# NekoImageLand/retto

Hardware: AMD Instinct MI355X
Metric: images/sec end-to-end PP-OCRv4 det+rec @960x960 (higher is better)
Workload: dtype f32; 1 GPU; C3: PP-OCRv4 mobile det+cls+rec full pipeline, batch=32 pages of 960x960 per GPU, 32 planted lines/page (planted DB map drives box extraction; det net fully executed, checksum 1.46374e+07); pages resident in HBM when the timed region starts; weights=seeded synthetic, PP-OCRv4 mobile shapes, networks=mobile/f32 f32 mobile/f32, parallelism=dp1 (pages sharded, no per-step collective), batches_in_flight=2

## Files before the change

### retto_amd/csrc/api_debug.cpp

```cpp
#include <cmath>
#include <cstdio>
#include <cstdlib>
#include <cstring>

#include "api_internal.h"

using namespace rt;

namespace {
using nh::half_t;

std::vector<half_t> pack_conv16_weights(const float* wt, int cout, int cin, int kh, int kw, int cin_pad) {
  const int npad = round_up(cout, 32), nslab = (cin_pad + nh::KS - 1) / nh::KS;
  std::vector<half_t> hw((size_t)nslab * kh * kw * npad * nh::KS, (half_t)0.f);
  for (int n = 0; n < cout; n++)
    for (int k = 0; k < cin; k++)
      for (int t = 0; t < kh * kw; t++)
        hw[(((size_t)(k / nh::KS) * kh * kw + t) * npad + n) * nh::KS + k % nh::KS] = (half_t)wt[((size_t)n * cin + k) * kh * kw + t];
  return hw;
}

inline uint64_t xorshift64(uint64_t& s) { s ^= s << 13; s ^= s >> 7; s ^= s << 17; return s; }

template <typename F>
// ... 234 lines not shown
    if (ctc >= 0) { DevBufs::download(idx_out, didx, (size_t)M); DevBufs::download(prob_out, dprob, (size_t)M); }
    plan_out[0] = (int)plan.kernel; plan_out[1] = plan.nt; plan_out[2] = plan.kg; plan_out[3] = plan.se; plan_out[4] = plan.bf;
  });
}

RT_API int rt_debug_dwconv(rt_session* s, const float* x, const int* heights, const int* widths, int n_img, int C, int Cp, int K,
                           int sh, int sw, const float* w, const float* bias, int act, int has_lab, float lab_a, float lab_c,
                           int pooled, int form, float* out, float* partial_out, long long partial_cap, float* mean_out,
                           int* info_out) {
  RT_REQUIRE(s && x && heights && widths && w && bias && out && info_out, s, "rt_debug_dwconv: null argument");
  RT_REQUIRE(n_img > 0 && C > 0 && Cp >= C && Cp % 4 == 0 && (K == 3 || K == 5) && sh >= 1 && sh <= 2 && sw >= 1 && sw <= 2 &&
                 act >= ACT_NONE && act <= ACT_SIGMOID && (form == 0 || form == 1),
             s, "rt_debug_dwconv: bad shape");
  RT_REQUIRE(!pooled || (partial_out && mean_out), s, "rt_debug_dwconv: pooled without buffers for the sums");
  for (int i = 0; i < n_img; i++) RT_REQUIRE(heights[i] > 0 && widths[i] > 0, s, "rt_debug_dwconv: empty image");
  const Ragged gi(heights, widths, n_img), go = gi.down(sh, sw);
  RT_REQUIRE(gi.total * Cp < (1ll << 30), s, "rt_debug_dwconv: too large");
  RestoreInt keep_form(nn::g_dw_sweep);
  nn::g_dw_sweep = form ? 4 : 0;
  const nn::DwPlan plan = nn::dw_plan(K, sh, sw, Cp, go.maxH, go.maxW, pooled != 0);
  const int chunks = pooled ? plan.chunks : 0, strip_R = pooled ? plan.R : 0, spb = pooled ? plan.spb : 0;
  const size_t npart = (size_t)n_img * chunks * Cp;
  RT_REQUIRE(!pooled || (long long)npart <= partial_cap, s, "rt_debug_dwconv: partial_out is too small");
  return guarded(s, [&] {
    RT_HIP_CHECK(hipSetDevice(s->device));
    DevBufs bufs;
    const size_t nout = (size_t)(go.total + 64) * Cp;
    const float *dx = bufs.upload(x, (size_t)gi.total * Cp), *dw = bufs.upload(w, (size_t)K * K * Cp), *db = bufs.upload(bias, (size_t)Cp);
    const ImgGeom *dgi = gi.upload(bufs), *dgo = go.upload(bufs);
    float* dy = bufs.canary<float>(nout, s->st);
    float* dpart = pooled ? bufs.canary<float>(npart, s->st) : nullptr;
    float* dmean = pooled ? bufs.alloc<float>((size_t)n_img * Cp) : nullptr;
    nn::dwconv(s->st, plan, dx, dgi, dgo, n_img, Cp, C, dw, db, act, has_lab, lab_a, lab_c, dy, dpart);
    if (pooled)
      nn::se_fc_from_dw(s->st, dpart, dgo, n_img, chunks, strip_R, spb, C, Cp, nullptr, nullptr, nullptr, nullptr, 0, 0.f, 0, dmean);
    RT_HIP_CHECK(hipStreamSynchronize(s->st));
    DevBufs::download(out, dy, nout);
    if (pooled) { DevBufs::download(partial_out, dpart, npart); DevBufs::download(mean_out, dmean, (size_t)n_img * Cp); }
    info_out[0] = chunks; info_out[1] = strip_R; info_out[2] = spb;
    info_out[3] = plan.kernel == nn::DwKernel::sweep ? 1 : 0;
  });
}

RT_API int rt_debug_attention(rt_session* s, const float* qkv, long long rows, const int* tokens, int n_lines, int heads, float* out) {
  RT_REQUIRE(s && qkv && tokens && out, s, "rt_debug_attention: null argument");
  RT_REQUIRE(rows > 0 && rows < (1ll << 30) && n_lines > 0 && heads > 0 && heads <= 64, s, "rt_debug_attention: bad shape");
  for (int i = 0; i < n_lines; i++) RT_REQUIRE(tokens[i] > 0, s, "rt_debug_attention: a line without tokens");
  const Ragged lines(tokens, n_lines);
  RT_REQUIRE(lines.total == rows, s, "rt_debug_attention: the lines' tokens do not add up to rows");
  return guarded(s, [&] {
    RT_HIP_CHECK(hipSetDevice(s->device));
    const int hd = 15, C = heads * hd;
    DevBufs bufs;
    const float* dq = bufs.upload(qkv, (size_t)rows * 3 * C);
    float* dout = bufs.zeroed<float>((size_t)rows * C);
    nn::attention(s->st, dq, lines.upload(bufs), n_lines, lines.maxW, heads, hd, dout);
    RT_HIP_CHECK(hipStreamSynchronize(s->st));
    DevBufs::download(out, dout, (size_t)rows * C);
  });
}

static LcBlock debug_lc_block(WeightStore& ws, int cin, int cout, int sh, int sw, const float* dw_w, const float* dw_bias, const float* pw_w,
                              const float* pw_bias, int dw_act, const Lab& dw_lab, const Lab& pw_lab) {
  LcBlock b;
  b.dw = pack_dw(ws, dw_w, dw_bias, cin, 3); b.dw_lab = dw_lab; b.dw_act = dw_act;
  b.pw = pack_conv(ws, pw_w, pw_bias, cout, cin, 1, 1); b.pw_lab = pw_lab;
  b.sh = sh; b.sw = sw; b.cin = cin; b.cout = cout;
  return b;
}
static float* debug_lc_mid(DevBufs& bufs, hipStream_t st, const LcBlock& b, const Level& Lo) {
  if (lc_block_plan(b, Lo).route != nn::LC_UNFUSED) return nullptr;
  const size_t nmid = (size_t)(Lo.total + 256) * b.dw.Cp;
  float* dy1 = bufs.alloc<float>(nmid);
  RT_HIP_CHECK(hipMemsetAsync(dy1, 0, nmid * sizeof(float), st));
  return dy1;
}

RT_API int rt_debug_lc_block(rt_session* s, const float* x, const int* heights, const int* widths, int n_img, int cin, int cout,
                             int sh, int sw, const float* dw_w, const float* dw_bias, const float* pw_w, const float* pw_bias,
                             int dw_act, int dw_has_lab, float dw_a, float dw_c, int pw_has_lab, float pw_a, float pw_c, int form,
                             float* out, int* info_out) {
  RT_REQUIRE(s && x && heights && widths && dw_w && dw_bias && pw_w && pw_bias && out && info_out, s, "rt_debug_lc_block: null argument");
  RT_REQUIRE(n_img > 0 && n_img <= RT_MAX_GRID_Y && cin > 0 && cout > 0 && chan_pitch(cin) == round_up(cin, 4) && sh >= 1 && sh <= 2 &&
                 sw >= 1 && sw <= 2 && dw_act >= ACT_NONE && dw_act <= ACT_SIGMOID && (form == 0 || form == 1 || form == 3),
             s, "rt_debug_lc_block: bad shape");
  const int Cp = chan_pitch(cin), ldy = chan_pitch(cout);
  std::vector<std::pair<int, int>> hw;
  for (int i = 0; i < n_img; i++) {
    RT_REQUIRE(heights[i] > 0 && widths[i] > 0, s, "rt_debug_lc_block: empty image");
    hw.push_back({heights[i], widths[i]});
  }
  Level Li = make_level(hw), Lo = down_level(Li, sh, sw);
  RT_REQUIRE(Li.total * Cp < (1ll << 30) && Lo.total * ldy < (1ll << 30), s, "rt_debug_lc_block: too large");
  return guarded(s, [&] {
    s->begin_call();
    WeightStore ws;
    const LcBlock b = debug_lc_block(ws, cin, cout, sh, sw, dw_w, dw_bias, pw_w, pw_bias, dw_act, Lab{dw_has_lab, dw_a, dw_c}, Lab{pw_has_lab, pw_a, pw_c});
    DevBufs bufs;
    RestoreInt keep_form(nn::g_lc_wave);
    nn::g_lc_wave = form;
    RunCtx c = s->ctx(&s->arena);
    upload_levels(c, {&Li, &Lo});
    const size_t nin = (size_t)Li.total * Cp, nout = (size_t)(Lo.total + 64) * ldy;
    const float* dx = bufs.upload(x, nin);
    float* dy = bufs.canary<float>(nout, s->st);
    run_lc(c, b, dx, Li, Lo, dy, debug_lc_mid(bufs, s->st, b, Lo));
    RT_HIP_CHECK(hipStreamSynchronize(s->st));
    DevBufs::download(out, dy, nout);
    info_out[0] = (int)lc_block_plan(b, Lo).route;
  });
}

RT_API int rt_debug_dw_plan(int K, int sh, int sw, int Cp, int maxHo, int maxWo, int pooled, int form, int* plan_out) {
  rt_session* const none = nullptr;
  RT_REQUIRE(plan_out, none, "rt_debug_dw_plan: null argument");
  RT_REQUIRE(Cp > 0 && Cp % 4 == 0 && maxHo > 0 && maxWo > 0 && (form == 0 || form == 1), none, "rt_debug_dw_plan: bad shape");
  RestoreInt keep_form(nn::g_dw_sweep);
  nn::g_dw_sweep = form ? 4 : 0;
  const nn::DwPlan p = nn::dw_plan(K, sh, sw, Cp, maxHo, maxWo, pooled != 0);
  const int f[8] = {(int)p.kernel, p.inst, p.R, p.lanes, p.spb, p.chunks, (int)p.grid_x, (int)p.grid_z};
  memcpy(plan_out, f, sizeof f);
  return RT_OK;
}

RT_API int rt_debug_lc_wide(rt_session* s, const float* x, const int* heights, const int* widths, int n_img, int K, int cin, int cout,
                            int sh, int sw, const float* dw_w, const float* dw_bias, const float* pw_w, const float* pw_bias, int dw_act,
                            int dw_has_lab, float dw_a, float dw_c, int pw_has_lab, float pw_a, float pw_c, const float* fc1_w,
                            const float* fc1_b, const float* fc2_w, const float* fc2_b, int dw_form, float* out, long long out_len,
                            float* y1_out, long long y1_len, float* scale_out, long long scale_len, int* info_out) {
  RT_REQUIRE(x && heights && widths && dw_w && dw_bias && pw_w && pw_bias && out && y1_out && info_out, s, "rt_debug_lc_wide: null argument");
  const bool se = fc1_w || fc1_b || fc2_w || fc2_b;
  RT_REQUIRE(!se || (fc1_w && fc1_b && fc2_w && fc2_b && scale_out), s, "rt_debug_lc_wide: a squeeze-excite block needs both FCs and scale_out");
  RT_REQUIRE(n_img > 0 && n_img <= 4096, s, "rt_debug_lc_wide: bad image count");
  RT_REQUIRE(cin > 0 && cin <= 512 && cin % 4 == 0 && cout > 0 && cout <= 960, s, "rt_debug_lc_wide: bad channel counts (cin a multiple of 4 up to 512, cout up to 960)");
  RT_REQUIRE((K == 3 || K == 5) && sh >= 1 && sh <= 2 && sw >= 1 && sw <= 2 && dw_act >= ACT_NONE && dw_act <= ACT_SIGMOID &&
                 (dw_form == 0 || dw_form == 1), s, "rt_debug_lc_wide: no such block (K 3 or 5, strides 1 or 2, dw_form 0 or 1)");
  for (int i = 0; i < n_img; i++)
    RT_REQUIRE(heights[i] > 0 && widths[i] > 0 && heights[i] <= 4096 && widths[i] <= 65536, s, "rt_debug_lc_wide: empty or oversized image");
  const int Cp = chan_pitch(cin), ldy = chan_pitch(cout);
  const Ragged gi(heights, widths, n_img), go = gi.down(sh, sw);
  RT_REQUIRE(gi.total * Cp < (1ll << 28) && go.total * ldy < (1ll << 28), s, "rt_debug_lc_wide: too large");
  const long long out_n = (go.total + 64) * ldy, y1_n = (go.total + 64) * Cp, scale_n = se ? (long long)(n_img + 64) * Cp : 0;
  RT_REQUIRE(out_len == out_n && y1_len == y1_n, s, "rt_debug_lc_wide: out or y1_out has the wrong length");
  RT_REQUIRE(scale_len == scale_n, s, "rt_debug_lc_wide: scale_out has the wrong length");
  RT_REQUIRE(s, s, "rt_debug_lc_wide: null session");
  return guarded(s, [&] {
    s->begin_call();
    WeightStore ws;
    LcBlock b;
    b.dw = pack_dw(ws, dw_w, dw_bias, cin, K); b.dw_lab = Lab{dw_has_lab, dw_a, dw_c}; b.dw_act = dw_act;
    b.se = se;
    if (se) b.sew = get_se(ws, fc1_w, fc1_b, fc2_w, fc2_b, cin, cin / 4);
    b.pw = pack_conv(ws, pw_w, pw_bias, cout, cin, 1, 1); b.pw_lab = Lab{pw_has_lab, pw_a, pw_c};
    b.sh = sh; b.sw = sw; b.cin = cin; b.cout = cout;
    std::vector<std::pair<int, int>> hw;
    for (int i = 0; i < n_img; i++) hw.push_back({heights[i], widths[i]});
    Level Li = make_level(hw), Lo = down_level(Li, sh, sw);
    DevBufs bufs;
    RestoreInt keep_form(nn::g_dw_sweep), keep_variant(nn::g_gemm_variant);
    nn::g_dw_sweep = dw_form ? 4 : 0;
    nn::g_gemm_variant = 0;
    RunCtx c = s->ctx(&s->arena);
    upload_levels(c, {&Li, &Lo});
    const float* dx = bufs.upload(x, (size_t)Li.total * Cp);
    float* dy = bufs.canary<float>((size_t)out_n, s->st);
    float* dy1 = bufs.canary<float>((size_t)(Lo.total + 256) * Cp, s->st);
    const nn::LcPlan plan = lc_block_plan(b, Lo);
    LcTrace tr;
    run_lc(c, b, dx, Li, Lo, dy, dy1, &tr);
    RT_HIP_CHECK(hipStreamSynchronize(s->st));
    DevBufs::download(out, dy, (size_t)out_n);
    DevBufs::download(y1_out, dy1, (size_t)y1_n);
    if (se) {
      const uint32_t cw = RT_DEBUG_CANARY;
      for (long long i = 0; i < scale_n; i++) memcpy(scale_out + i, &cw, 4);
      if (tr.scale) DevBufs::download(scale_out, tr.scale, (size_t)n_img * Cp);
    }
    const bool unfused = plan.route == nn::LC_UNFUSED;
    const int f[16] = {(int)plan.route, unfused ? (int)plan.dw.kernel : 0, unfused ? plan.dw.inst : plan.inst, plan.dw.R, plan.dw.lanes,
                       plan.dw.spb, plan.dw.chunks, (int)plan.dw.grid_x, (int)plan.dw.grid_z, plan.se_rows,
                       unfused ? (int)tr.gemm.kernel : 0, unfused && tr.gemm.se ? 1 : 0, tr.scale ? (tr.scaled_in_place ? 2 : 1) : 0, 0, 0, 0};
    memcpy(info_out, f, sizeof f);
  });
// ... 567 lines not shown
      x_need = gi.total * Cp; out_rows = go.total;
      break;
    case G32_AVGPOOL:
      ldy = ip[1];
      ok = C % 4 == 0 && ldy >= C && ldy <= 16384 && ldy % 4 == 0;
      for (int i = 0; ok && i < n_img; i++) ok = heights[i] >= 3 && widths[i] >= 2;
      if (ok) go = gi.pool(3, 2);
      x_need = gi.total * Cp; out_rows = go.total;
      break;
    case G32_SOFTMAX: case G32_ARGMAX_PROB: case G32_ARGMAX:
      ok = ip[1] >= C && ip[1] <= 16384 && (op == G32_SOFTMAX || idx_out);
      x_need = (long long)n_img * ip[1]; out_rows = n_img; ldy = op == G32_SOFTMAX ? C : 1;
      break;
  }
  RT_REQUIRE(ok, s, "rt_debug_glue32: bad parameters for the op");
  RT_REQUIRE(x_need < (1ll << 28) && out_rows * ldy < (1ll << 28), s, "rt_debug_glue32: too large");
  const long long out_n = (out_rows + 64) * ldy;
  RT_REQUIRE(x_len >= x_need && out_len == out_n, s, "rt_debug_glue32: x is too short or out has the wrong length");
  RT_REQUIRE(out2_n == 0 || (out2 && out2_len == out2_n), s, "rt_debug_glue32: out2 is missing or has the wrong length");
  RT_REQUIRE(s, s, "rt_debug_glue32: null session");
  return guarded(s, [&] {
    RT_HIP_CHECK(hipSetDevice(s->device));
    DevBufs bufs;
    WeightStore ws;
    hipStream_t st = s->st;
    float* dout = bufs.canary<float>((size_t)out_n, st);
    const ImgGeom* dgi = rows_op ? nullptr : gi.upload(bufs);
    switch (op) {
      case G32_SE_SCALE: {
        const SeW se = get_se(ws, w[0], w[1], w[2], w[3], C, Cr);
        float* dx = nullptr;
        if (out2_n) { dx = bufs.canary<float>((size_t)out2_n, st); DevBufs::put(dx, x, (size_t)x_need); }
        else dx = bufs.upload(x, (size_t)x_need);
        float* partial = bufs.alloc<float>((size_t)n_img * nn::pool_chunks(gi.max_pix) * Cp);
        nn::se_scale(st, dx, dgi, n_img, gi.max_pix, se.C, Cp, se.w1, se.b1, se.w2, se.b2, se.Cr, fp[0], ip[2], partial, dout);
        if (out2_n) nn::scale_channels(st, dx, dgi, n_img, gi.max_pix, Cp, dout);
        RT_HIP_CHECK(hipStreamSynchronize(st));
        if (out2_n) DevBufs::download(out2, dx, (size_t)out2_n);
      } break;
      case G32_GLOBAL_MEAN: {
        float* partial = bufs.alloc<float>((size_t)n_img * nn::pool_chunks(gi.max_pix) * Cp);
        nn::global_mean(st, bufs.upload(x, (size_t)x_need), dgi, n_img, gi.max_pix, Cp, partial, dout);
      } break;
      case G32_MAXPOOL: nn::maxpool_2x2(st, bufs.upload(x, (size_t)x_need), dgi, go.upload(bufs), n_img, go.max_pix, Cp, dout); break;
      case G32_AVGPOOL: nn::avgpool_3x2(st, bufs.upload(x, (size_t)x_need), dgi, go.upload(bufs), n_img, go.max_pix, Cp, dout, ldy); break;
      case G32_SOFTMAX: nn::softmax_rows(st, bufs.upload(x, (size_t)x_need), ip[1], n_img, C, dout); break;
      case G32_ARGMAX_PROB: case G32_ARGMAX: {
        int* didx = bufs.canary<int>((size_t)out_n, st);
        const float* dx = bufs.upload(x, (size_t)x_need);
        if (op == G32_ARGMAX_PROB) nn::argmax_prob_rows(st, dx, ip[1], n_img, C, didx, dout);
        else nn::argmax_rows(st, dx, ip[1], n_img, C, didx, dout);
        RT_HIP_CHECK(hipStreamSynchronize(st));
        DevBufs::download(idx_out, didx, (size_t)out_n);
      } break;
    }
    RT_HIP_CHECK(hipStreamSynchronize(st));
    DevBufs::download(out, dout, (size_t)out_n);
  });
}

RT_API int rt_bench_lc(rt_session* s, int n, int h, int w, int cin, int cout, int stride, int form, int iters, float* ms_out, float* maxdiff_out) {
  RT_REQUIRE(s && ms_out && n > 0 && h > 0 && w > 0 && cin > 0 && cout > 0 && (stride == 1 || stride == 2 || stride == 21), s, "rt_bench_lc: bad argument");
  return guarded(s, [&] {
    s->begin_call();
    const int sh = stride == 21 ? 2 : stride, sw = stride == 21 ? 1 : stride;
    std::vector<float> hwd((size_t)cin * 9), hbd(cin), hw((size_t)cout * cin), hb(cout);
    uint32_t st = 777;
    auto rnd = [&]() { st = st * 1664525u + 1013904223u; return ((st >> 8) & 0xffff) / 32768.0f - 1.0f; };
    for (auto& v : hwd) v = rnd() * 0.3f;
    for (auto& v : hw) v = rnd() * 0.1f;
    for (auto& v : hbd) v = rnd() * 0.1f;
    for (auto& v : hb) v = rnd() * 0.2f;
    const bool plain_tail = sh == 2 && sw == 2;
    WeightStore ws;
    const LcBlock blk = debug_lc_block(ws, cin, cout, sh, sw, hwd.data(), hbd.data(), hw.data(), hb.data(), plain_tail ? ACT_NONE : ACT_HSWISH,
                                     Lab{!plain_tail, 0.99f, 0.01f}, Lab{1, 1.01f, 0.02f});
    Level Li = make_level(std::vector<std::pair<int, int>>((size_t)n, {h, w})), Lo = down_level(Li, sh, sw);
    RunCtx c = s->ctx(&s->arena);
    upload_levels(c, {&Li, &Lo});
    const size_t nin = (size_t)Li.total * blk.dw.Cp, nout = (size_t)Lo.total * chan_pitch(cout);
    std::vector<float> hx(nin, 0.f);
    for (size_t p = 0; p < (size_t)Li.total; p++) for (int k = 0; k < cin; k++) hx[p * blk.dw.Cp + k] = rnd();
    DevBufs bufs;
    RestoreInt keep_form(nn::g_lc_wave);
    float *dx = bufs.upload(hx.data(), nin), *dy = bufs.zeroed<float>(nout), *dy0 = bufs.zeroed<float>(nout);
    float* dy1 = nullptr;
    auto run = [&](float* out) {
      if (!dy1) dy1 = debug_lc_mid(bufs, s->st, blk, Lo);
      run_lc(c, blk, dx, Li, Lo, out, dy1);
    };
    nn::g_lc_wave = 0; run(dy0);
    nn::g_lc_wave = form;
    timed_and_compared(s->st, iters, [&] { run(dy); }, dy0, dy, nout, ms_out, maxdiff_out);
  });
}

RT_API int rt_debug_det_tiles(rt_session* s, const uint8_t* rgb_det, int h, int w, float* tile_maps_out, float* page_map_out) {
  RT_REQUIRE(s && rgb_det && page_map_out, s, "rt_debug_det_tiles: null argument");
  return guarded(s, [&] { s->debug_det_tiles(rgb_det, h, w, tile_maps_out, page_map_out); });
}
RT_API int rt_debug_rec_windows(rt_session* s, const float* nchw, int n, const int* widths, int32_t* unit_idx_out, float* unit_prob_out,
                                float* unit_z5_out, int32_t* line_idx_out, float* line_prob_out, float* line_z5_out) {
  RT_REQUIRE(s && nchw && widths && n > 0, s, "rt_debug_rec_windows: bad argument");
  return guarded(s, [&] {
    s->debug_rec_windows(nchw, n, widths, unit_idx_out, unit_prob_out, unit_z5_out, line_idx_out, line_prob_out, line_z5_out);
  });
}
RT_API int rt_debug_arena_high_water(rt_session* s, long long* out3) {
  RT_REQUIRE(s && out3, s, "rt_debug_arena_high_water: null argument");
  return guarded(s, [&] {
    out3[0] = (long long)s->arena.high_water(); out3[1] = (long long)s->scratch.high_water(); out3[2] = (long long)s->dbws.high_water();
  });
}
RT_API int rt_bench_memcpy_d2d(rt_session* s, size_t bytes, int iters, float* ms_out) {
  RT_REQUIRE(s && ms_out && bytes > 0 && iters > 0, s, "rt_bench_memcpy_d2d: bad argument");
  return guarded(s, [&] {
    RT_HIP_CHECK(hipSetDevice(s->device));
    DevBufs bufs;
    char* a = bufs.zeroed<char>(bytes); char* b = bufs.zeroed<char>(bytes);
    Events ev;
    RT_HIP_CHECK(hipEventCreate(&ev.a)); RT_HIP_CHECK(hipEventCreate(&ev.b));
    RT_HIP_CHECK(hipMemcpyAsync(b, a, bytes, hipMemcpyDeviceToDevice, s->st));
    RT_HIP_CHECK(hipEventRecord(ev.a, s->st));
    for (int i = 0; i < iters; i++) RT_HIP_CHECK(hipMemcpyAsync(b, a, bytes, hipMemcpyDeviceToDevice, s->st));
    RT_HIP_CHECK(hipEventRecord(ev.b, s->st));
    RT_HIP_CHECK(hipStreamSynchronize(s->st));
    float ms = 0.f;
    RT_HIP_CHECK(hipEventElapsedTime(&ms, ev.a, ev.b));
    *ms_out = ms / (float)iters;
  });
}

}
```

### retto_amd/csrc/lc_plan.cpp

```cpp
#include "lc_plan.h"

#include "gemm_plan.h"

namespace rt {
namespace nn {

int g_lc_wave = env_int("RT_LC_WAVE", 3);
int g_dw_sweep = env_int("RT_DW_SWEEP", 4);

namespace {

struct SweepInst { int K, sh, sw, min_ho, inst, inst_pooled; };
constexpr SweepInst SWEEPS[] = {{5, 1, 1, 5, 1, 3}, {3, 1, 1, 3, 2, 0}, {5, 2, 1, 3, 4, 5}, {3, 1, 2, 3, 6, 0}};

struct ThinInst { int sh, sw, c4, nt32, inst, th; };
constexpr ThinInst THINS[] = {{1, 1, 4, 1, 1, 8},  {1, 1, 8, 2, 2, 8},
                              {1, 1, 12, 2, 3, 4}, {1, 1, 16, 2, 4, 4},
                              {2, 2, 8, 2, 6, 4},  {2, 2, 12, 3, 7, 4}};
struct WaveInst { int sh, sw, Cp, Npad16, inst; };
constexpr WaveInst WAVES[] = {{1, 1, 16, 32, 1}, {1, 1, 32, 64, 2}, {1, 1, 48, 48, 3}, {1, 1, 64, 64, 4},
                              {2, 2, 32, 48, 6}, {2, 2, 48, 96, 7}, {2, 1, 64, 128, 8}};

int thin_inst(const LcShape& s, int* th) {
  if (s.K != 3 || s.Cp != round_up(s.C, 4)) return 0;
  for (const ThinInst& t : THINS)
    if (t.sh == s.sh && t.sw == s.sw && t.c4 * 4 == s.Cp && t.nt32 == (s.Npad16 + 31) / 32) { *th = t.th; return t.inst; }
  return 0;
}

int wave_inst(const LcShape& s, const Epilogue& epi) {
  if (s.K != 3 || s.Cp != s.C || s.N != s.Npad16) return 0;
  if (epi.residual || epi.a_scale || epi.am_max || !epi.bias || epi.act != ACT_HSWISH) return 0;
  if (!epi.has_lab) return 0;
  const bool plain_tail = s.sh == 2 && s.sw == 2;
  if (plain_tail ? (s.dw_act != ACT_NONE || s.dw_has_lab) : (s.dw_act != ACT_HSWISH || !s.dw_has_lab)) return 0;
  const long long in_bytes = (long long)(s.maxHo * s.sh + 2) * (s.maxWo * s.sw + 2) * s.Cp * 4;
  const long long out_bytes = (long long)s.maxHo * s.maxWo * s.ldy * 4;
  if (in_bytes >= (1ll << 30) || out_bytes >= (1ll << 30)) return 0;
  for (const WaveInst& w : WAVES)
    if (w.sh == s.sh && w.sw == s.sw && w.Cp == s.Cp && w.Npad16 == s.Npad16) return w.inst;
  return 0;
}

}

DwPlan dw_plan(int K, int sh, int sw, int Cp, int maxHo, int maxWo, bool pooled) {
  DwPlan p;
  if ((K != 3 && K != 5) || sh < 1 || sh > 2 || sw < 1 || sw > 2) return p;
  p.R = (maxHo == 6 || (maxHo == 3 && sh == 1)) ? 3 : (sh == 1 ? 4 : 2);
  const bool wide = K == 5 ? Cp >= 192 && (sw == 1 || (sh == 2 && p.R == 2)) : Cp >= 128 && sh == 1 && p.R == 4 && !pooled;
  p.lanes = wide ? 16 : 8;
  p.spb = 256 / p.lanes;
  const int strips_x = (maxWo + 3) / 4, strips_y = (maxHo + p.R - 1) / p.R;
  p.chunks = (int)(((long long)strips_x * strips_y + p.spb - 1) / p.spb);
  p.grid_z = (unsigned)((Cp + p.lanes * 4 - 1) / (p.lanes * 4));
  if (g_dw_sweep && wide && maxHo * sh <= 24)
    for (const SweepInst& s : SWEEPS)
      if (s.K == K && s.sh == sh && s.sw == sw && maxHo >= s.min_ho) {
        const bool pool3 = p.R == 3 && strips_y <= DW_SWEEP_POOL_STRIPS;
        p.inst = !pooled ? s.inst : pool3 ? s.inst_pooled : 0;
      }
  if (p.inst) {
    p.kernel = DwKernel::sweep;
    p.grid_x = (unsigned)((strips_x + p.spb - 1) / p.spb);
  } else {
    p.kernel = wide ? DwKernel::rows64 : DwKernel::rows32;
    p.inst = dw_rows_inst(p.lanes, K, p.R, sh, sw);
    p.grid_x = (unsigned)p.chunks;
  }
  return p;
}

LcPlan lc_plan(const LcShape& s, const Epilogue& epi) {
  LcPlan p;
  const int tiles_x = (s.maxWo + 15) / 16;
  auto fused = [&](LcRoute route, int inst, int tile_h, int tiles_per_block) {
    p.route = route; p.inst = inst; p.tile_h = tile_h;
    p.grid_x = (unsigned)((tiles_x * ((s.maxHo + tile_h - 1) / tile_h) + tiles_per_block - 1) / tiles_per_block);
    return p;
  };
  if (!s.se) {
    int th = 0;
    if (const int inst = g_lc_wave ? wave_inst(s, epi) : 0) {
      if (g_lc_wave >= 3 || inst >= 6) return fused(LC_LDS, inst, s.sh == 1 ? 4 : 2, 4 * LC_WAVE_TPW);
      return fused(LC_WAVE, inst, 2, 4 * LC_WAVE_TPW);
    }
    if (const int inst = thin_inst(s, &th)) return fused(LC_THIN, inst, th, LC_THIN_TPB);
  }
  if (s.se && (s.K == 3 || s.K == 5))
    p.se_rows = gemm_se_rows(s.Cp, s.rows, round_up(s.C, 4), s.N, s.Npad16, epi.act, s.min_pix);
  p.dw = dw_plan(s.K, s.sh, s.sw, s.Cp, s.maxHo, s.maxWo, p.se_rows > 0);
  return p;
}

}
}
```

### retto_amd/csrc/lc_plan.h

```cpp
#pragma once
#include "common.h"

namespace rt {
namespace nn {

extern int g_lc_wave;
extern int g_dw_sweep;

constexpr int DW_SWEEP_POOL_STRIPS = 4;
constexpr int LC_THIN_TPB = 8;
constexpr int LC_WAVE_TPW = 4;

constexpr int dw_rows_inst(int lanes, int K, int R, int sh, int sw) { return (((lanes * 8 + K) * 8 + R) * 4 + sh) * 4 + sw; }
enum class DwKernel {
  invalid,
  rows32,
  rows64,
  sweep,
};
struct DwPlan {
  DwKernel kernel = DwKernel::invalid;
  int inst = 0;
  int R = 0;
  int lanes = 0;
  int spb = 0;
  int chunks = 0;
  unsigned grid_x = 0, grid_z = 0;
};
DwPlan dw_plan(int K, int sh, int sw, int Cp, int maxHo, int maxWo, bool pooled);

enum LcRoute { LC_UNFUSED = 0, LC_THIN = 1, LC_WAVE = 2, LC_LDS = 3 };
struct LcShape {
  int K = 3, sh = 1, sw = 1;
  int Cp = 0, C = 0;
  int N = 0, Npad16 = 0;
  int dw_act = ACT_NONE, dw_has_lab = 0;
  bool se = false;
  int maxHo = 0, maxWo = 0, ldy = 0;
  long long rows = 0, min_pix = 0;
};
struct LcPlan {
  LcRoute route = LC_UNFUSED;
  int inst = 0, tile_h = 0;
  unsigned grid_x = 0;
  DwPlan dw;
  int se_rows = 0;
};
LcPlan lc_plan(const LcShape& s, const Epilogue& epi);

}
}
```

### retto_amd/csrc/nn_lcwave.hip

```cpp
#include "common.h"
#include "nn_dev.h"

namespace rt {
namespace nn {

namespace {
constexpr int LROW = KC + 4;
constexpr int DPP_ROW_SHL1 = 0x101, DPP_ROW_SHR1 = 0x111;

template <int CTRL>
__device__ __forceinline__ f32x4 dpp_row(const f32x4& old, const f32x4& src) {
  f32x4 o;
#pragma unroll
  for (int e = 0; e < 4; e++) {
    const float fo = old[e], fs = src[e];
    o[e] = __int_as_float(__builtin_amdgcn_update_dpp(__float_as_int(fo), __float_as_int(fs), CTRL, 0xf, 0xf, false));
  }
  return o;
}
}

typedef float f32x2 __attribute__((ext_vector_type(2)));

__device__ __forceinline__ f32x4 hswish_lab4(const f32x4& v, float lab_a, float lab_c) {
  f32x4 t = v + 3.0f;
#pragma unroll
  for (int e = 0; e < 4; e++) { const float te = t[e]; t[e] = __builtin_amdgcn_fmed3f(te, 0.0f, 6.0f); }
  f32x4 o = v * t;
  o = o * 0.16666667f;
  const f32x4 a4 = {lab_a, lab_a, lab_a, lab_a}, c4 = {lab_c, lab_c, lab_c, lab_c};
  return __builtin_elementwise_fma(o, a4, c4);
}

struct LcwArgs {
  const float* x; const ImgGeom* gin; const ImgGeom* gout;
  const float* Wd; const float* bd; const float* Wp; const float* bias; float* y;
  float dw_a, dw_c, pw_a, pw_c;
  int Npad, ldy, tiles_per_wave;
};

template <int G, int NT, int MT, bool DWA>
__global__ __launch_bounds__(256) __attribute__((amdgpu_waves_per_eu(3, 3))) void k_lc_wave(LcwArgs p) {
  constexpr int CP = G * 16, NKC = (CP + KC - 1) / KC, NCOL = NT * 16;
  constexpr int IR = MT + 2;
  constexpr int NV = 2;
  __shared__ __attribute__((aligned(16))) float wt[NKC * NCOL * LROW];
  __shared__ __attribute__((aligned(16))) float tp[10 * CP + NCOL];
  const ImgGeom g = p.gout[blockIdx.y], gi = p.gin[blockIdx.y];
  const int tiles_x = (g.W + 15) / 16, tiles_y = (g.H + MT - 1) / MT, n_tiles = tiles_x * tiles_y;
  const int first = blockIdx.x * 4 * p.tiles_per_wave;
  if (first >= n_tiles) return;
  const int tid = threadIdx.x, lane = tid & 63, wave = __builtin_amdgcn_readfirstlane(tid >> 6), r = lane & 15, q = lane >> 4;
  for (int idx = tid; idx < NKC * NCOL * 8; idx += 256) {
    const int c4i = idx & 7, row = (idx >> 3) % NCOL, kc = (idx >> 3) / NCOL;
    *reinterpret_cast<f32x4*>(wt + (kc * NCOL + row) * LROW + c4i * 4) =
        *reinterpret_cast<const f32x4*>(p.Wp + ((long long)kc * p.Npad + row) * KC + c4i * 4);
  }
  for (int idx = tid; idx < 10 * CP / 4; idx += 256)
    *reinterpret_cast<f32x4*>(tp + idx * 4) =
        idx < 9 * CP / 4 ? *reinterpret_cast<const f32x4*>(p.Wd + idx * 4) : *reinterpret_cast<const f32x4*>(p.bd + (idx - 9 * CP / 4) * 4);
  for (int idx = tid; idx < NCOL / 4; idx += 256) *reinterpret_cast<f32x4*>(tp + 10 * CP + idx * 4) = *reinterpret_cast<const f32x4*>(p.bias + idx * 4);
  __syncthreads();

  const __amdgpu_buffer_rsrc_t xrs = __builtin_amdgcn_make_buffer_rsrc(
      const_cast<float*>(p.x + gi.off * CP), 0, (unsigned)gi.H * (unsigned)gi.W * (CP * 4), 0x00020000);
  const __amdgpu_buffer_rsrc_t yrs = __builtin_amdgcn_make_buffer_rsrc(
      p.y + g.off * p.ldy, 0, (unsigned)g.H * (unsigned)g.W * (unsigned)p.ldy * 4, 0x00020000);
  const unsigned row_bytes = (unsigned)gi.W * CP * 4, yrow_bytes = (unsigned)g.W * (unsigned)p.ldy * 4;
  constexpr unsigned OOB = 0x80000000u;

  int tile = first + wave;
  if (tile >= n_tiles) return;
  int ty = tile / tiles_x, tx = tile - ty * tiles_x;
  ty = __builtin_amdgcn_readfirstlane(ty); tx = __builtin_amdgcn_readfirstlane(tx);

  f32x4 in[IR][NV];
  unsigned c_off, h_off, y_off;
  auto lane_offsets = [&](int txx) __attribute__((always_inline)) {
    const int ox = txx * 16 + r, ix = ox;
    const int hx = r == 0 ? ox - 1 : ox + 1;
    const bool h_ok = (r == 0 || r == 15) && (unsigned)hx < (unsigned)gi.W;
    c_off = ix < gi.W ? (unsigned)ix * (CP * 4) + q * 16 : OOB;
    h_off = h_ok ? (unsigned)hx * (CP * 4) + q * 16 : OOB;
    y_off = ox < g.W ? (unsigned)ox * ((unsigned)p.ldy * 4) + q * 16 : OOB;
  };
  const bool edge_lane = r == 0 || r == 15;
  auto fetch = [&](int tyy, auto gg_tag) __attribute__((always_inline)) {
    constexpr int GG = decltype(gg_tag)::value;
#pragma unroll
    for (int i = 0; i < IR; i++) {
      const int iy = tyy * MT - 1 + i;
      if ((unsigned)iy < (unsigned)gi.H) {
        const unsigned so = (unsigned)iy * row_bytes + GG * 64;
        in[i][0] = __builtin_bit_cast(f32x4, __builtin_amdgcn_raw_buffer_load_b128(xrs, c_off, so, 0));
      } else {
#pragma unroll
        for (int v = 0; v < NV - 1; v++) in[i][v] = f32x4{0.f, 0.f, 0.f, 0.f};
      }
    }
    if (edge_lane) {
#pragma unroll
      for (int i = 0; i < IR; i++) {
        const int iy = tyy * MT - 1 + i;
        if ((unsigned)iy < (unsigned)gi.H) in[i][NV - 1] = __builtin_bit_cast(f32x4, __builtin_amdgcn_raw_buffer_load_b128(xrs, h_off, (unsigned)iy * row_bytes + GG * 64, 0));
        else in[i][NV - 1] = f32x4{0.f, 0.f, 0.f, 0.f};
      }
    }
  };

  lane_offsets(tx);
  fetch(ty, IntTag<0>{});
  for (int it = 0; it < p.tiles_per_wave; it++) {
    int ntx = tx + 4, nty = ty;
    while (ntx >= tiles_x) { ntx -= tiles_x; nty++; }
    const bool more = it + 1 < p.tiles_per_wave && nty < tiles_y;
    const unsigned y_off_t = y_off;
    f32x4 acc[MT][NT];
#pragma unroll
    for (int gg = 0; gg < G; gg++) {
      f32x4 a[MT];
      {
// ... 143 lines not shown
#pragma unroll
    for (int gg = 0; gg < G; gg++) {
      const int b = DEPTH == 2 ? (gg & 1) : 0;
#pragma unroll
      for (int j = 0; j < NJ; j++) *reinterpret_cast<__attribute__((address_space(3))) f32x4*>(wr[j] & 0x1ffff) = st[b][j];
      __builtin_amdgcn_sched_barrier(0);
      {
        const int nx = gg + DEPTH;
        if (nx < G) {
          switch (nx) {
            case 1: fetch(IntTag<1 % G>{}, IntTag<(1 % G) % DEPTH>{}); break;
            case 2: fetch(IntTag<2 % G>{}, IntTag<(2 % G) % DEPTH>{}); break;
            case 3: fetch(IntTag<3 % G>{}, IntTag<(3 % G) % DEPTH>{}); break;
            case 4: fetch(IntTag<4 % G>{}, IntTag<(4 % G) % DEPTH>{}); break;
            case 5: fetch(IntTag<5 % G>{}, IntTag<(5 % G) % DEPTH>{}); break;
            case 6: fetch(IntTag<6 % G>{}, IntTag<(6 % G) % DEPTH>{}); break;
            default: fetch(IntTag<7 % G>{}, IntTag<(7 % G) % DEPTH>{}); break;
          }
        } else if (more) {
          if (nx == G) lane_offsets(nty, ntx);
          if (nx == G) fetch(IntTag<0>{}, IntTag<0>{}); else fetch(IntTag<1 % G>{}, IntTag<DEPTH - 1>{});
        }
      }
      __builtin_amdgcn_sched_barrier(0);
      f32x4 a[MT];
      {
        const float* tq = tp + (4 * gg + q) * 4;
        f32x4 dsum[MT];
        const f32x4 dwb = *reinterpret_cast<const f32x4*>(tq + 9 * CP);
#pragma unroll
        for (int mt = 0; mt < MT; mt++) dsum[mt] = dwb;
#pragma unroll
        for (int i = 0; i < IR; i++) {
          f32x4 col[3];
#pragma unroll
          for (int dx = 0; dx < 3; dx++) col[dx] = *reinterpret_cast<const f32x4*>(rd[dx] + i * RP);
#pragma unroll
          for (int mt = 0; mt < MT; mt++) {
            const int dy = i - mt * SH;
            if (dy < 0 || dy > 2) continue;
#pragma unroll
            for (int dx = 0; dx < 3; dx++) {
              const f32x4 w = *reinterpret_cast<const f32x4*>(tq + (dy * 3 + dx) * CP);
              dsum[mt] = __builtin_elementwise_fma(col[dx], w, dsum[mt]);
            }
          }
        }
#pragma unroll
        for (int mt = 0; mt < MT; mt++) a[mt] = DWA ? hswish_lab4(dsum[mt], p.dw_a, p.dw_c) : dsum[mt];
      }
      __builtin_amdgcn_sched_barrier(0);
      const float* wg = wt + ((gg >> 1) * NCOL + r) * LROW + (gg & 1) * 16 + 4 * q;
#pragma unroll
      for (int nt = 0; nt < NT; nt++) {
        const f32x4 b = *reinterpret_cast<const f32x4*>(wg + nt * 16 * LROW);
#pragma unroll
        for (int s = 0; s < 4; s++)
#pragma unroll
          for (int mt = 0; mt < MT; mt++) {
            if (gg == 0 && s == 0) acc[mt][nt] = __builtin_amdgcn_mfma_f32_16x16x4f32(b[s], a[mt][s], f32x4{0.f, 0.f, 0.f, 0.f}, 0, 0, 0);
            else acc[mt][nt] = __builtin_amdgcn_mfma_f32_16x16x4f32(b[s], a[mt][s], acc[mt][nt], 0, 0, 0);
          }
      }
      __builtin_amdgcn_sched_barrier(0);
    }
#pragma unroll
    for (int mt = 0; mt < MT; mt++) {
      const int oy = ty * MT + mt;
      if (oy < g.H) {
        const unsigned y_row = y_off_t == OOB ? OOB : y_off_t + (unsigned)oy * yrow_bytes;
#pragma unroll
        for (int nt = 0; nt < NT; nt++) {
          const f32x4 bias = *reinterpret_cast<const f32x4*>(tp + 10 * CP + nt * 16 + q * 4);
          const f32x4 o = hswish_lab4(acc[mt][nt] + bias, p.pw_a, p.pw_c);
          __builtin_amdgcn_raw_buffer_store_b128(__builtin_bit_cast(__attribute__((ext_vector_type(4))) unsigned, o), yrs, y_row + nt * 64, 0, 0);
        }
      }
    }
    if (!more) break;
    tx = ntx; ty = nty;
  }
}

void lc_wave(hipStream_t st, const LcPlan& p, const float* x, const ImgGeom* gin, const ImgGeom* gout, int n_img, int C,
             const float* Wd, const float* bd, int dw_act, int dw_has_lab, float dw_a, float dw_c, const float* Wp, int N, int Npad16,
             float* y, int ldy, const Epilogue& epi) {
  if (n_img <= 0) return;
  const dim3 grid(p.grid_x, n_img);
  const LcwArgs a{x, gin, gout, Wd, bd, Wp, epi.bias, y, dw_a, dw_c, epi.has_lab ? epi.lab_a : 1.f, epi.has_lab ? epi.lab_c : 0.f, Npad16, ldy, LC_WAVE_TPW};
#define RT_LCL(INST, GG, NN, MT, S1, S2, DWA) case 10 * LC_LDS + INST: RT_LAUNCH((k_lc_lds<GG, NN, MT, S1, S2, DWA, 2>), grid, dim3(256), 0, st, a); return;
#define RT_LCW(INST, GG, NN) case 10 * LC_WAVE + INST: RT_LAUNCH((k_lc_wave<GG, NN, 2, true>), grid, dim3(256), 0, st, a); return;
  switch (10 * p.route + p.inst) {
    RT_LCL(1, 1, 2, 4, 1, 1, true) RT_LCL(2, 2, 4, 4, 1, 1, true) RT_LCL(3, 3, 3, 4, 1, 1, true) RT_LCL(4, 4, 4, 4, 1, 1, true)
    RT_LCL(6, 2, 3, 2, 2, 2, false) RT_LCL(7, 3, 6, 2, 2, 2, false) RT_LCL(8, 4, 8, 2, 2, 1, true)
    RT_LCW(1, 1, 2) RT_LCW(2, 2, 4) RT_LCW(3, 3, 3) RT_LCW(4, 4, 4)
  }
#undef RT_LCW
#undef RT_LCL
  throw RtError(8, "lc_wave: the plan names no k_lc_lds / k_lc_wave instance");
}

}
}
```

Baseline: 1242 images/s.

## Add strip-walking fused dw+pw kernel that reuses halo rows down short images

Adds a k_lc_strip kernel and an LC_STRIP plan route for fused depthwise-3x3 plus pointwise blocks on short feature maps, such as the recognition lines. Each wave walks a vertical strip of tiles and keeps the overlapping input rows from the tile above in LDS instead of reloading them from global memory. Each block packs several images, and the next group's loads are double-buffered. The aim is to cut redundant input traffic and improve occupancy for small-height layers, at the cost of more LDS per block, serial work along a strip, and a new heuristic for choosing the segment length.

```diff
diff --git a/retto_amd/csrc/api_debug.cpp b/retto_amd/csrc/api_debug.cpp
--- a/retto_amd/csrc/api_debug.cpp
+++ b/retto_amd/csrc/api_debug.cpp
@@ -340,7 +340,7 @@
                              float* out, int* info_out) {
   RT_REQUIRE(s && x && heights && widths && dw_w && dw_bias && pw_w && pw_bias && out && info_out, s, "rt_debug_lc_block: null argument");
   RT_REQUIRE(n_img > 0 && n_img <= RT_MAX_GRID_Y && cin > 0 && cout > 0 && chan_pitch(cin) == round_up(cin, 4) && sh >= 1 && sh <= 2 &&
-                 sw >= 1 && sw <= 2 && dw_act >= ACT_NONE && dw_act <= ACT_SIGMOID && (form == 0 || form == 1 || form == 3),
+                 sw >= 1 && sw <= 2 && dw_act >= ACT_NONE && dw_act <= ACT_SIGMOID && (form == 0 || form == 1 || form == 3 || form == 4),
              s, "rt_debug_lc_block: bad shape");
   const int Cp = chan_pitch(cin), ldy = chan_pitch(cout);
   std::vector<std::pair<int, int>> hw;
@@ -355,8 +355,8 @@
     WeightStore ws;
     const LcBlock b = debug_lc_block(ws, cin, cout, sh, sw, dw_w, dw_bias, pw_w, pw_bias, dw_act, Lab{dw_has_lab, dw_a, dw_c}, Lab{pw_has_lab, pw_a, pw_c});
     DevBufs bufs;
-    RestoreInt keep_form(nn::g_lc_wave);
-    nn::g_lc_wave = form;
+    RestoreInt keep_form(nn::g_lc_wave), keep_strip(nn::g_lc_strip);
+    nn::g_lc_wave = form == 4 ? 3 : form; nn::g_lc_strip = form == 4;
     RunCtx c = s->ctx(&s->arena);
     upload_levels(c, {&Li, &Lo});
     const size_t nin = (size_t)Li.total * Cp, nout = (size_t)(Lo.total + 64) * ldy;
@@ -1090,15 +1090,16 @@
     std::vector<float> hx(nin, 0.f);
     for (size_t p = 0; p < (size_t)Li.total; p++) for (int k = 0; k < cin; k++) hx[p * blk.dw.Cp + k] = rnd();
     DevBufs bufs;
-    RestoreInt keep_form(nn::g_lc_wave);
+    RestoreInt keep_form(nn::g_lc_wave), keep_strip(nn::g_lc_strip);
     float *dx = bufs.upload(hx.data(), nin), *dy = bufs.zeroed<float>(nout), *dy0 = bufs.zeroed<float>(nout);
+    RT_HIP_CHECK(hipDeviceSynchronize());
     float* dy1 = nullptr;
     auto run = [&](float* out) {
       if (!dy1) dy1 = debug_lc_mid(bufs, s->st, blk, Lo);
       run_lc(c, blk, dx, Li, Lo, out, dy1);
     };
     nn::g_lc_wave = 0; run(dy0);
-    nn::g_lc_wave = form;
+    nn::g_lc_wave = form == 4 ? 3 : form; nn::g_lc_strip = form == 4;
     timed_and_compared(s->st, iters, [&] { run(dy); }, dy0, dy, nout, ms_out, maxdiff_out);
   });
 }
diff --git a/retto_amd/csrc/lc_plan.cpp b/retto_amd/csrc/lc_plan.cpp
--- a/retto_amd/csrc/lc_plan.cpp
+++ b/retto_amd/csrc/lc_plan.cpp
@@ -6,6 +6,7 @@
 namespace nn {
 
 int g_lc_wave = env_int("RT_LC_WAVE", 3);
+int g_lc_strip = -1;
 int g_dw_sweep = env_int("RT_DW_SWEEP", 4);
 
 namespace {
@@ -20,6 +21,24 @@
 struct WaveInst { int sh, sw, Cp, Npad16, inst; };
 constexpr WaveInst WAVES[] = {{1, 1, 16, 32, 1}, {1, 1, 32, 64, 2}, {1, 1, 48, 48, 3}, {1, 1, 64, 64, 4},
                               {2, 2, 32, 48, 6}, {2, 2, 48, 96, 7}, {2, 1, 64, 128, 8}};
+
+struct StripInst { int inst, max_ho; };
+constexpr StripInst STRIPS[] = {{1, 24}, {2, 24}, {3, 0}, {4, 24}, {8, 12}};
+constexpr int LC_STRIP_MAX_SEG = 16;
+
+int strip_seg(const LcShape& s, int inst, int tile_h) {
+  const StripInst* si = nullptr;
+  for (const StripInst& t : STRIPS) if (t.inst == inst) si = &t;
+  if (!si || g_lc_strip == 0) return 0;
+  const int tiles_y = (s.maxHo + tile_h - 1) / tile_h, cap = tiles_y < LC_STRIP_MAX_SEG ? tiles_y : LC_STRIP_MAX_SEG;
+  const bool force = g_lc_strip > 0;
+  if (!force && (s.maxHo > si->max_ho || tiles_y < 2)) return 0;
+  const long long strips = (s.rows / s.maxHo + 15) / 16;
+  const long long by_cap = (tiles_y + cap - 1) / cap, by_waves = (LC_STRIP_ROUNDS + strips - 1) / strips;
+  const long long n = by_cap > by_waves ? by_cap : by_waves;
+  const int seg = (int)((tiles_y + n - 1) / n);
+  return seg >= 2 ? seg : force ? cap : 0;
+}
 
 int thin_inst(const LcShape& s, int* th) {
   if (s.K != 3 || s.Cp != round_up(s.C, 4)) return 0;
@@ -82,7 +101,15 @@
   if (!s.se) {
     int th = 0;
     if (const int inst = g_lc_wave ? wave_inst(s, epi) : 0) {
-      if (g_lc_wave >= 3 || inst >= 6) return fused(LC_LDS, inst, s.sh == 1 ? 4 : 2, 4 * LC_WAVE_TPW);
+      if (g_lc_wave >= 3 || inst >= 6) {
+        const int tile_h = s.sh == 1 ? 4 : 2;
+        if (const int seg = strip_seg(s, inst, tile_h)) {
+          p.route = LC_STRIP; p.inst = inst; p.tile_h = tile_h; p.seg = seg;
+          p.grid_x = (unsigned)((LC_STRIP_IMGS * tiles_x * ((s.maxHo + tile_h * seg - 1) / (tile_h * seg)) + 3) / 4);
+          return p;
+        }
+        return fused(LC_LDS, inst, tile_h, 4 * LC_WAVE_TPW);
+      }
       return fused(LC_WAVE, inst, 2, 4 * LC_WAVE_TPW);
     }
     if (const int inst = thin_inst(s, &th)) return fused(LC_THIN, inst, th, LC_THIN_TPB);
diff --git a/retto_amd/csrc/lc_plan.h b/retto_amd/csrc/lc_plan.h
--- a/retto_amd/csrc/lc_plan.h
+++ b/retto_amd/csrc/lc_plan.h
@@ -5,11 +5,14 @@
 namespace nn {
 
 extern int g_lc_wave;
+extern int g_lc_strip;
 extern int g_dw_sweep;
 
 constexpr int DW_SWEEP_POOL_STRIPS = 4;
 constexpr int LC_THIN_TPB = 8;
 constexpr int LC_WAVE_TPW = 4;
+constexpr int LC_STRIP_IMGS = 4;
+constexpr int LC_STRIP_ROUNDS = 2 * 2048;
 
 constexpr int dw_rows_inst(int lanes, int K, int R, int sh, int sw) { return (((lanes * 8 + K) * 8 + R) * 4 + sh) * 4 + sw; }
 enum class DwKernel {
@@ -29,7 +32,7 @@
 };
 DwPlan dw_plan(int K, int sh, int sw, int Cp, int maxHo, int maxWo, bool pooled);
 
-enum LcRoute { LC_UNFUSED = 0, LC_THIN = 1, LC_WAVE = 2, LC_LDS = 3 };
+enum LcRoute { LC_UNFUSED = 0, LC_THIN = 1, LC_WAVE = 2, LC_LDS = 3, LC_STRIP = 4 };
 struct LcShape {
   int K = 3, sh = 1, sw = 1;
   int Cp = 0, C = 0;
@@ -41,7 +44,7 @@
 };
 struct LcPlan {
   LcRoute route = LC_UNFUSED;
-  int inst = 0, tile_h = 0;
+  int inst = 0, tile_h = 0, seg = 0;
   unsigned grid_x = 0;
   DwPlan dw;
   int se_rows = 0;
diff --git a/retto_amd/csrc/nn_lcwave.hip b/retto_amd/csrc/nn_lcwave.hip
--- a/retto_amd/csrc/nn_lcwave.hip
+++ b/retto_amd/csrc/nn_lcwave.hip
@@ -36,7 +36,7 @@
   const float* x; const ImgGeom* gin; const ImgGeom* gout;
   const float* Wd; const float* bd; const float* Wp; const float* bias; float* y;
   float dw_a, dw_c, pw_a, pw_c;
-  int Npad, ldy, tiles_per_wave;
+  int Npad, ldy, tiles_per_wave, n_img;
 };
 
 template <int G, int NT, int MT, bool DWA>
@@ -346,23 +346,232 @@
   }
 }
 
+template <int G, int NT, int MT, int SH, bool DWA, int WPE>
+__global__ __launch_bounds__(256) __attribute__((amdgpu_waves_per_eu(WPE, WPE))) void k_lc_strip(LcwArgs p) {
+  constexpr int CP = G * 16, NKC = (CP + KC - 1) / KC, NCOL = NT * 16;
+  constexpr int KEEP = 3 - SH, NR = MT * SH, IR = KEEP + NR, PXR = 18, RP = PXR * 64;
+  static_assert(IR == (MT - 1) * SH + 3 && NR >= KEEP, "a tile's rows = the rows kept from the tile above + MT * SH new ones");
+  constexpr int SLOTS = NR * PXR * 4, NJ = (SLOTS + 63) / 64;
+  constexpr int HSLOTS = KEEP * G * PXR * 4, NH = (HSLOTS + 63) / 64;
+  constexpr int KS0 = (NR - KEEP) * PXR * 4, JK = KS0 / 64;
+  constexpr int HB = KEEP * G * RP, XB = HB + NR * RP + 512;
+  __shared__ __attribute__((aligned(16))) float wt[NKC * NCOL * LROW];
+  __shared__ __attribute__((aligned(16))) float tp[10 * CP + NCOL];
+  __shared__ __attribute__((aligned(16))) char xb[4 * XB];
+  const int seg = p.tiles_per_wave;
+  const int img0 = blockIdx.y * LC_STRIP_IMGS, img1 = min(img0 + LC_STRIP_IMGS, p.n_img);
+  auto segments = [&](int i) { const ImgGeom t = p.gout[i]; return ((t.W + 15) / 16) * (((t.H + MT - 1) / MT + seg - 1) / seg); };
+  {
+    int total = 0;
+    for (int i = img0; i < img1; i++) total += segments(i);
+    if ((int)blockIdx.x * 4 >= total) return;
+  }
+  const int tid = threadIdx.x, lane = tid & 63, wave = __builtin_amdgcn_readfirstlane(tid >> 6), r = lane & 15, q = lane >> 4;
+  const int n0 = blockIdx.z * NCOL;
+  for (int idx = tid; idx < NKC * NCOL * 8; idx += 256) {
+    const int c4i = idx & 7, row = (idx >> 3) % NCOL, kc = (idx >> 3) / NCOL;
+    *reinterpret_cast<f32x4*>(wt + (kc * NCOL + row) * LROW + c4i * 4) =
+        *reinterpret_cast<const f32x4*>(p.Wp + ((long long)kc * p.Npad + n0 + row) * KC + c4i * 4);
+  }
+  for (int idx = tid; idx < 10 * CP / 4; idx += 256)
+    *reinterpret_cast<f32x4*>(tp + idx * 4) =
+        idx < 9 * CP / 4 ? *reinterpret_cast<const f32x4*>(p.Wd + idx * 4) : *reinterpret_cast<const f32x4*>(p.bd + (idx - 9 * CP / 4) * 4);
+  for (int idx = tid; idx < NCOL / 4; idx += 256) *reinterpret_cast<f32x4*>(tp + 10 * CP + idx * 4) = *reinterpret_cast<const f32x4*>(p.bias + n0 + idx * 4);
+  __syncthreads();
+
+  int sid = blockIdx.x * 4 + wave, img = img0;
+  for (; img < img1; img++) {
+    const int n = segments(img);
+    if (sid < n) break;
+    sid -= n;
+  }
+  if (img >= img1) return;
+  img = __builtin_amdgcn_readfirstlane(img); sid = __builtin_amdgcn_readfirstlane(sid);
+  const ImgGeom g = p.gout[img], gi = p.gin[img];
+  const int tiles_x = (g.W + 15) / 16, tiles_y = (g.H + MT - 1) / MT;
+  const __amdgpu_buffer_rsrc_t xrs = __builtin_amdgcn_make_buffer_rsrc(
+      const_cast<float*>(p.x + gi.off * CP), 0, (unsigned)gi.H * (unsigned)gi.W * (CP * 4), 0x00020000);
+  const __amdgpu_buffer_rsrc_t yrs = __builtin_amdgcn_make_buffer_rsrc(
+      p.y + g.off * p.ldy, 0, (unsigned)g.H * (unsigned)g.W * (unsigned)p.ldy * 4, 0x00020000);
+  const unsigned row_bytes = (unsigned)gi.W * CP * 4, yrow_bytes = (unsigned)g.W * (unsigned)p.ldy * 4;
+  constexpr unsigned OOB = 0x80000000u;
+
+  int sy = sid / tiles_x, tx = sid - sy * tiles_x;
+  sy = __builtin_amdgcn_readfirstlane(sy); tx = __builtin_amdgcn_readfirstlane(tx);
+  const int ty0 = sy * seg, ty1 = min(ty0 + seg, tiles_y);
+
+  char* const xw = xb + wave * XB;
+  const unsigned xw_lds = (unsigned)(size_t)(__attribute__((address_space(3))) char*)xw;
+  auto swz = [](int px, int c) { return (px * 4 + (c ^ ((px >> 1) & 3))) * 16; };
+  auto pix_off = [&](int px, int c) -> unsigned {
+    const int ix = tx * 16 - 1 + px;
+    return (unsigned)ix < (unsigned)gi.W ? (unsigned)ix * (CP * 4) + c * 16 : OOB;
+  };
+  f32x4 hst[NH];
+  unsigned hwr[NH];
+#pragma unroll
+  for (int j = 0; j < NH; j++) {
+    const int t = lane + 64 * j, k = t / (G * PXR * 4), rem = t - k * (G * PXR * 4), gg = rem / (PXR * 4), rem2 = rem - gg * (PXR * 4);
+    const int px = rem2 >> 2, c = rem2 & 3, iy = ty0 * NR - 1 + k;
+    const unsigned po = pix_off(px, c);
+    const bool ok = t < HSLOTS && po != OOB && (unsigned)iy < (unsigned)gi.H;
+    hwr[j] = xw_lds + (t < HSLOTS ? (k * G + gg) * RP + swz(px, c) : HB + NR * RP + (lane & 31) * 16);
+    hst[j] = __builtin_bit_cast(f32x4, __builtin_amdgcn_raw_buffer_load_b128(xrs, ok ? (unsigned)iy * row_bytes + po + gg * 64 : OOB, 0, 0));
+  }
+  unsigned wr[NJ], coff[NJ];
+#pragma unroll
+  for (int j = 0; j < NJ; j++) {
+    const int t = lane + 64 * j, row = t / (PXR * 4), rem = t - row * (PXR * 4), px = rem >> 2, c = rem & 3;
+    wr[j] = (xw_lds + (t < SLOTS ? HB + row * RP + swz(px, c) : HB + NR * RP + (lane & 31) * 16)) | (unsigned)(t < SLOTS ? row : 63) << 25;
+    coff[j] = t < SLOTS ? pix_off(px, c) : OOB;
+  }
+  unsigned kwr[NJ - JK];
+  bool kept[NJ - JK];
+#pragma unroll
+  for (int j = JK; j < NJ; j++) {
+    const int t = lane + 64 * j, row = t / (PXR * 4), rem = t - row * (PXR * 4), px = rem >> 2, c = rem & 3;
+    kept[j - JK] = t >= KS0 && t < SLOTS;
+    kwr[j - JK] = xw_lds + (row - (NR - KEEP)) * G * RP + swz(px, c);
+  }
+  const char* rd[3];
+#pragma unroll
+  for (int dx = 0; dx < 3; dx++) rd[dx] = xw + swz(r + dx, q);
+
+  constexpr int DEPTH = (MT == 4 && G % 2 == 0 && SH == 1) ? 2 : 1;
+  unsigned goff[NJ];
+  f32x4 st[DEPTH][NJ];
+  auto lane_offsets = [&](int tyy) __attribute__((always_inline)) {
+#pragma unroll
+    for (int j = 0; j < NJ; j++) {
+      const int iy = tyy * NR - 1 + KEEP + (int)(wr[j] >> 25);
+      goff[j] = coff[j] != OOB && iy < gi.H ? (unsigned)iy * row_bytes + coff[j] : OOB;
+    }
+  };
+  auto fetch = [&](auto gg_tag, auto buf_tag) __attribute__((always_inline)) {
+    constexpr int GG = decltype(gg_tag)::value, B = decltype(buf_tag)::value;
+#pragma unroll
+    for (int j = 0; j < NJ; j++) st[B][j] = __builtin_bit_cast(f32x4, __builtin_amdgcn_raw_buffer_load_b128(xrs, goff[j], GG * 64, 0));
+  };
+  const int ox = tx * 16 + r;
+  const unsigned y_off = ox < g.W ? (unsigned)ox * ((unsigned)p.ldy * 4) + n0 * 4 + q * 16 : OOB;
+
+  lane_offsets(ty0);
+  fetch(IntTag<0>{}, IntTag<0>{});
+  if (DEPTH == 2) fetch(IntTag<1 % G>{}, IntTag<DEPTH - 1>{});
+#pragma unroll
+  for (int j = 0; j < NH; j++) *reinterpret_cast<__attribute__((address_space(3))) f32x4*>(hwr[j]) = hst[j];
+  __builtin_amdgcn_sched_barrier(0);
+
+  for (int ty = ty0; ty < ty1; ty++) {
+    const bool more = ty + 1 < ty1;
+    f32x4 acc[MT][NT];
+#pragma unroll
+    for (int gg = 0; gg < G; gg++) {
+      const int b = DEPTH == 2 ? (gg & 1) : 0;
+#pragma unroll
+      for (int j = 0; j < NJ; j++) *reinterpret_cast<__attribute__((address_space(3))) f32x4*>(wr[j] & 0x1ffff) = st[b][j];
+      f32x4 hcol[KEEP][3];
+#pragma unroll
+      for (int i = 0; i < KEEP; i++)
+#pragma unroll
+        for (int dx = 0; dx < 3; dx++) hcol[i][dx] = *reinterpret_cast<const f32x4*>(rd[dx] + (i * G + gg) * RP);
+      __builtin_amdgcn_sched_barrier(0);
+#pragma unroll
+      for (int j = JK; j < NJ; j++)
+        if (kept[j - JK]) *reinterpret_cast<__attribute__((address_space(3))) f32x4*>(kwr[j - JK] + gg * RP) = st[b][j];
+      __builtin_amdgcn_sched_barrier(0);
+      {
+        const int nx = gg + DEPTH;
+        if (nx < G) {
+          switch (nx) {
+            case 1: fetch(IntTag<1 % G>{}, IntTag<(1 % G) % DEPTH>{}); break;
+            case 2: fetch(IntTag<2 % G>{}, IntTag<(2 % G) % DEPTH>{}); break;
+            default: fetch(IntTag<3 % G>{}, IntTag<(3 % G) % DEPTH>{}); break;
+          }
+        } else if (more) {
+          if (nx == G) lane_offsets(ty + 1);
+          if (nx == G) fetch(IntTag<0>{}, IntTag<0>{}); else fetch(IntTag<1 % G>{}, IntTag<DEPTH - 1>{});
+        }
+      }
+      __builtin_amdgcn_sched_barrier(0);
+      f32x4 a[MT];
+      {
+        const float* tq = tp + (4 * gg + q) * 4;
+        f32x4 dsum[MT];
+        const f32x4 dwb = *reinterpret_cast<const f32x4*>(tq + 9 * CP);
+#pragma unroll
+        for (int mt = 0; mt < MT; mt++) dsum[mt] = dwb;
+#pragma unroll
+        for (int i = 0; i < IR; i++) {
+          f32x4 col[3];
+#pragma unroll
+          for (int dx = 0; dx < 3; dx++) col[dx] = i < KEEP ? hcol[i < KEEP ? i : 0][dx] : *reinterpret_cast<const f32x4*>(rd[dx] + HB + (i - KEEP) * RP);
+#pragma unroll
+          for (int mt = 0; mt < MT; mt++) {
+            const int dy = i - mt * SH;
+            if (dy < 0 || dy > 2) continue;
+#pragma unroll
+            for (int dx = 0; dx < 3; dx++) {
+              const f32x4 w = *reinterpret_cast<const f32x4*>(tq + (dy * 3 + dx) * CP);
+              dsum[mt] = __builtin_elementwise_fma(col[dx], w, dsum[mt]);
+            }
+          }
+        }
+#pragma unroll
+        for (int mt = 0; mt < MT; mt++) a[mt] = DWA ? hswish_lab4(dsum[mt], p.dw_a, p.dw_c) : dsum[mt];
+      }
+      __builtin_amdgcn_sched_barrier(0);
+      const float* wg = wt + ((gg >> 1) * NCOL + r) * LROW + (gg & 1) * 16 + 4 * q;
+#pragma unroll
+      for (int nt = 0; nt < NT; nt++) {
+        const f32x4 bw = *reinterpret_cast<const f32x4*>(wg + nt * 16 * LROW);
+#pragma unroll
+        for (int s = 0; s < 4; s++)
+#pragma unroll
+          for (int mt = 0; mt < MT; mt++) {
+            if (gg == 0 && s == 0) acc[mt][nt] = __builtin_amdgcn_mfma_f32_16x16x4f32(bw[s], a[mt][s], f32x4{0.f, 0.f, 0.f, 0.f}, 0, 0, 0);
+            else acc[mt][nt] = __builtin_amdgcn_mfma_f32_16x16x4f32(bw[s], a[mt][s], acc[mt][nt], 0, 0, 0);
+          }
+      }
+      __builtin_amdgcn_sched_barrier(0);
+    }
+#pragma unroll
+    for (int mt = 0; mt < MT; mt++) {
+      const int oy = ty * MT + mt;
+      if (oy < g.H) {
+        const unsigned y_row = y_off == OOB ? OOB : y_off + (unsigned)oy * yrow_bytes;
+#pragma unroll
+        for (int nt = 0; nt < NT; nt++) {
+          const f32x4 bias = *reinterpret_cast<const f32x4*>(tp + 10 * CP + nt * 16 + q * 4);
+          const f32x4 o = hswish_lab4(acc[mt][nt] + bias, p.pw_a, p.pw_c);
+          __builtin_amdgcn_raw_buffer_store_b128(__builtin_bit_cast(__attribute__((ext_vector_type(4))) unsigned, o), yrs, y_row + nt * 64, 0, 0);
+        }
+      }
+    }
+  }
+}
+
 void lc_wave(hipStream_t st, const LcPlan& p, const float* x, const ImgGeom* gin, const ImgGeom* gout, int n_img, int C,
              const float* Wd, const float* bd, int dw_act, int dw_has_lab, float dw_a, float dw_c, const float* Wp, int N, int Npad16,
              float* y, int ldy, const Epilogue& epi) {
   if (n_img <= 0) return;
-  const dim3 grid(p.grid_x, n_img);
-  const LcwArgs a{x, gin, gout, Wd, bd, Wp, epi.bias, y, dw_a, dw_c, epi.has_lab ? epi.lab_a : 1.f, epi.has_lab ? epi.lab_c : 0.f, Npad16, ldy, LC_WAVE_TPW};
+  const dim3 grid(p.grid_x, p.route == LC_STRIP ? (n_img + LC_STRIP_IMGS - 1) / LC_STRIP_IMGS : n_img);
+  const LcwArgs a{x, gin, gout, Wd, bd, Wp, epi.bias, y, dw_a, dw_c, epi.has_lab ? epi.lab_a : 1.f, epi.has_lab ? epi.lab_c : 0.f, Npad16, ldy,
+                  p.route == LC_STRIP ? p.seg : LC_WAVE_TPW, n_img};
 #define RT_LCL(INST, GG, NN, MT, S1, S2, DWA) case 10 * LC_LDS + INST: RT_LAUNCH((k_lc_lds<GG, NN, MT, S1, S2, DWA, 2>), grid, dim3(256), 0, st, a); return;
+#define RT_LCS(INST, GG, NN, MT, S1) case 10 * LC_STRIP + INST: RT_LAUNCH((k_lc_strip<GG, NN, MT, S1, true, 2>), grid, dim3(256), 0, st, a); return;
 #define RT_LCW(INST, GG, NN) case 10 * LC_WAVE + INST: RT_LAUNCH((k_lc_wave<GG, NN, 2, true>), grid, dim3(256), 0, st, a); return;
   switch (10 * p.route + p.inst) {
+    RT_LCS(1, 1, 2, 4, 1) RT_LCS(2, 2, 4, 4, 1) RT_LCS(3, 3, 3, 4, 1) RT_LCS(4, 4, 4, 4, 1) RT_LCS(8, 4, 8, 2, 2)
     RT_LCL(1, 1, 2, 4, 1, 1, true) RT_LCL(2, 2, 4, 4, 1, 1, true) RT_LCL(3, 3, 3, 4, 1, 1, true) RT_LCL(4, 4, 4, 4, 1, 1, true)
     RT_LCL(6, 2, 3, 2, 2, 2, false) RT_LCL(7, 3, 6, 2, 2, 2, false) RT_LCL(8, 4, 8, 2, 2, 1, true)
     RT_LCW(1, 1, 2) RT_LCW(2, 2, 4) RT_LCW(3, 3, 3) RT_LCW(4, 4, 4)
   }
 #undef RT_LCW
+#undef RT_LCS
 #undef RT_LCL
-  throw RtError(8, "lc_wave: the plan names no k_lc_lds / k_lc_wave instance");
-}
-
-}
-}
+  throw RtError(8, "lc_wave: the plan names no k_lc_lds / k_lc_strip / k_lc_wave instance");
+}
+
+}
+}
```

Result: no change. 1242 images/s (-0.0%).
